# unclearness/vacancy

Measured on AMD Instinct MI355X. Metric: Mvoxel*views/s (Carve), higher is better.
Workload: dtype f32

## Files before the change

vacancy_amd/csrc/carve_fused.h:

```cpp
#pragma once
#include <algorithm>
#include <cstdint>

#include "carve_common.h"
#include "carve_fused_plan.h"

namespace vcy {

constexpr int kMaxFusedViews = 64;
constexpr int kTileRaw = 16;
constexpr int kRawBuffers = 2;
template <int TQ>
constexpr int tile_f4_per_wave() { return TQ == kTileRaw ? kRawBuffers * 64 : TQ; }
constexpr int kTileBig = 512;
constexpr int kBigPixels = 4 * kTileBig;

constexpr int kCoopSdfPitch = 8 * VCY_WG_WAVES + 4;
template <typename CountT>
constexpr int coop_cnt_pitch() { return 8 * VCY_WG_WAVES + 16 / (int)sizeof(CountT); }
template <typename CountT>
constexpr size_t coop_lds_bytes() {
  return 64 * (size_t)kCoopSdfPitch * sizeof(float) + 64 * (size_t)coop_cnt_pitch<CountT>() * sizeof(CountT) +
         2 * VCY_WG_WAVES * sizeof(unsigned long long);
}

template <typename CountT, int NB>
constexpr size_t row_lds_bytes_per_wave() {
  return (size_t)kRawBuffers * 1024 + (size_t)NB * kRowMaxViews * 56  +
         (size_t)NB * 64 * WX * (sizeof(float) + sizeof(CountT)) + (size_t)NB * sizeof(unsigned long long);
}

#ifndef VCY_FAST_GROUP
#define VCY_FAST_GROUP 4
#endif
#ifndef VCY_WAVES
#define VCY_WAVES 7
#endif
#ifndef VCY_WAVES_CHECKED
#define VCY_WAVES_CHECKED 5
#endif
#ifndef VCY_WAVES_WA
#define VCY_WAVES_WA 6
#endif
#ifndef VCY_WAVES_WA_ONE
#define VCY_WAVES_WA_ONE 7
#endif
#ifndef VCY_WAVES_ONE
#define VCY_WAVES_ONE 8
#endif

struct FusedView {
  ViewParams v;
  const float* wmax;
  int wmax_plane;
  int has_lower;
  int wrect[4];
};
constexpr int kC0Stride = 32;

struct TileInfo {
  float lo_x, hi_x, lo_y, hi_y;
  float pitchf;
  int base;
  int tx0, ty0, tw, nq;
  int th;
  float inv_tw;
  float ub;
  int sure;
};
static_assert(sizeof(TileInfo) == 56, "row_lds_bytes_per_wave");

struct FootprintRecord {
  uint32_t w0, w1;
};
static_assert(sizeof(FootprintRecord) == kFootprintRecordBytes, "plan_fused_launch's chunk size");

__device__ __forceinline__ uint32_t pack_footprint_ub(float ub) {
  uint32_t b = __float_as_uint(ub);
  if (!(fabsf(ub) <= 3.402823466e+38f)) b = 0x7f800000u;
  else if (b & 0x80000000u) b &= ~63u;
  else b = (b + 63u) & ~63u;
  return b;
}

__device__ __forceinline__ FootprintRecord pack_footprint(const TileInfo& ti, const ViewParams& v) {
  const uint32_t b = pack_footprint_ub(ti.ub);
  FootprintRecord r;
  const int tx1 = ti.tx0 + ti.tw - 1, ty1 = ti.ty0 + ti.th - 1;
  r.w0 = b | (uint32_t)ti.th | (ti.nq && tx1 == v.roi_max_xi ? 16u : 0u) | (ti.nq && ty1 == v.roi_max_yi ? 32u : 0u);
  r.w1 = ti.nq ? ((uint32_t)ti.tx0 | ((uint32_t)ti.ty0 << 13) | ((uint32_t)ti.tw << 26) | ((uint32_t)ti.sure << 30)) : 0u;
// ... 166 lines not shown
```

vacancy_amd/csrc/carve_fused.hip:

```cpp
#include <algorithm>
#include <cmath>
#include <cstddef>
#include <cstdlib>
#include <cstring>
#include <map>
#include <mutex>
#include <utility>
#include <vector>

#include "carve_fused_device.h"

namespace vcy {
namespace {

constexpr int kWmaxPlanes = 2;


__device__ __forceinline__ void wmax_load8(const float* __restrict__ row, int x0, int w, bool vec, float a[8]) {
#pragma unroll
  for (int j = 0; j < 8; ++j) a[j] = -INFINITY;
  if (row == nullptr) return;
  if (vec) {
    const float4 lo = *(const float4*)(row + x0);
    a[0] = lo.x, a[1] = lo.y, a[2] = lo.z, a[3] = lo.w;
// ... 205 lines not shown
namespace {
__global__ __launch_bounds__(256) void c0_records_kernel(const FusedView* __restrict__ views, const float* __restrict__ px,
                                                         int nx, int nbw, float* __restrict__ c2) {
  const int t = blockIdx.x * 256 + threadIdx.x;
  const int b = t >> 3, k = t & 7;
  if (b >= nbw) return;
  const ViewParams& v = views[blockIdx.y].v;
  const float p = px[min(b * WX + k, nx - 1)];
  float* rec = c2 + ((size_t)blockIdx.y * nbw + b) * kC0Stride;
  rec[2 * k + 0] = v.r[0][0] * p;
  rec[2 * k + 1] = v.r[1][0] * p;
  rec[16 + k] = v.r[2][0] * p;
  rec[24 + k] = 0.0f;
}
}

bool fused_eligible(const vcy_ctx* c, int n_views, const vcy_view* views) {
  const vcy_update_option& u = c->opt.update_option;
  if (count_width_for(c, c->st.views_carved + n_views) > 2) return false;
  if (u.voxel_update == VCY_UPDATE_WEIGHTED_AVERAGE && !sane(u.voxel_update_weight)) return false;
  if (!carve_offsets_fit_32(std::min(n_views, kMaxFusedViews), (c->nx + WX - 1) / WX)) return false;
  for (int i = 0; i < n_views; ++i) {
    const vcy_view& v = views[i];
    if (v.is_ortho != views[0].is_ortho) return false;
    if (!v.is_ortho && (!sane(v.fx) || !sane(v.fy))) return false;
    if (v.width > 8192 || v.height > 8192) return false;
  }
  return true;
}

bool FusedViewCache::matches(const FusedViewKey& k, const void* vp_now, size_t vp_bytes) const {
  return valid && vp.size() == vp_bytes && std::memcmp(vp.data(), vp_now, vp_bytes) == 0 && key == k;
}
void FusedViewCache::remember(const FusedViewKey& k, const void* vp_now, size_t vp_bytes, bool samef_now, int max_quads_now) {
  vp.assign((const char*)vp_now, (const char*)vp_now + vp_bytes);
  key = k, samef = samef_now, max_quads = max_quads_now;
  valid = true;
}

int FusedViewStage::next(size_t bytes, void** out) {
  if (h[1].bytes() < bytes) {
    for (int q = 0; q < 2; ++q) {
      if (ev[q]) (void)hipEventSynchronize(ev[q]);
      (void)h[q].reset();
    }
    const size_t room = bytes + bytes / 2 + 4096;
    for (int q = 0; q < 2; ++q) {
      VCY_HIP_CHECK(ev[q].ensure(hipEventDisableTiming));
      VCY_HIP_CHECK(h[q].alloc(room));
    }
  }
  idx ^= 1;
  VCY_HIP_CHECK(hipEventSynchronize(ev[idx]));
  *out = h[idx];
  return VCY_OK;
}
int FusedViewStage::copied(hipStream_t stream) {
  VCY_HIP_CHECK(hipEventRecord(ev[idx], stream));
  return VCY_OK;
}

struct PreparedViews {
  float* d_c2;
  FusedView* d_views;
  bool samef;
  int max_quads;
};

namespace {

void fill_view_blocks(const vcy_ctx* c, int n_views, const ViewParams* vp, bool ortho, bool need_bound, bool need_lower,
                      int zlo, int zhi, FusedView* fv, bool* samef_out, int* max_quads_out) {
  std::memset((void*)fv, 0, sizeof(FusedView) * (size_t)n_views);
  bool samef = true;
  for (int vi = 0; vi < n_views; ++vi) {
    fv[vi].v = vp[vi];
    samef = samef && (vp[vi].fx == vp[vi].fy);
  }
  int max_quads = 0;
  if (need_bound && c->fused.d_wmax) {
    const int planes = need_lower ? 2 * kWmaxPlanes : kWmaxPlanes;
    const double X[2] = {c->h_px_min, c->h_px_max}, Y[2] = {c->h_py_min, c->h_py_max};
    const double Z[2] = {c->h_pz[zlo], c->h_pz[zhi - 1]};
    size_t off = 0;
    for (int vi = 0; vi < n_views; ++vi) {
      const int npx = vp[vi].width * vp[vi].height;
      fv[vi].wmax = c->fused.d_wmax + off;
      fv[vi].wmax_plane = npx;
      fv[vi].has_lower = need_lower ? 1 : 0;
      off += ((size_t)planes * npx + 3) & ~(size_t)3;
      const ImageRect r = slab_image_rect(vp[vi], ortho, X, Y, Z, vp[vi].width, vp[vi].height);
      for (int i = 0; i < 4; ++i) fv[vi].wrect[i] = r.wrect[i];
      max_quads = std::max(max_quads, r.quads);
    }
  }
  *samef_out = samef, *max_quads_out = max_quads;
}

}

int prepare_views(vcy_ctx* c, int n_views, const ViewParams* vp, bool ortho, bool need_bound, bool need_lower, int zlo,
                  int zhi, PreparedViews* out) {
  FusedState& f = c->fused;
  const int nxp = (c->nx + WX - 1) / WX * WX, nbw = nxp / WX;
  const size_t c2_bytes = (size_t)n_views * nbw * kC0Stride * sizeof(float);
  const size_t fv_bytes = sizeof(FusedView) * (size_t)n_views;
  const size_t vp_bytes = sizeof(ViewParams) * (size_t)n_views;
  if (need_bound) {
    const int planes = need_lower ? 2 * kWmaxPlanes : kWmaxPlanes;
    size_t total = 0;
    for (int vi = 0; vi < n_views; ++vi) total += ((size_t)planes * vp[vi].width * vp[vi].height + 3) & ~(size_t)3;
    if (f.d_wmax.bytes() < total * sizeof(float)) {
      VCY_HIP_CHECK(hipStreamSynchronize(c->stream));
      if (f.d_wmax.alloc(total * sizeof(float)) != hipSuccess) (void)hipGetLastError();
    }
  }
  {
    const size_t had = f.d_scratch.bytes();
    const hipError_t eg = f.d_scratch.grow(c2_bytes + fv_bytes, c->stream);
    if (eg != hipSuccess || f.d_scratch.bytes() != had) f.cache.valid = false;
    VCY_HIP_CHECK(eg);
  }
  float* d_c2 = (float*)f.d_scratch;
  FusedView* d_views = (FusedView*)((char*)f.d_scratch + c2_bytes);
  const FusedViewKey key{f.d_wmax, (void*)d_c2, need_bound, need_lower, ortho, zlo, zhi};
  if (!f.cache.matches(key, vp, vp_bytes)) {
    static_assert(kC0Stride == 32 && WX == 8, "c0_records_kernel's record layout");
    void* stage = nullptr;
    { const int rcs = f.stage.next(fv_bytes, &stage); if (rcs != VCY_OK) return rcs; }
    bool samef = true;
    int max_quads = 0;
    fill_view_blocks(c, n_views, vp, ortho, need_bound, need_lower, zlo, zhi, (FusedView*)stage, &samef, &max_quads);
    VCY_HIP_CHECK(hipMemcpyAsync(d_views, stage, fv_bytes, hipMemcpyHostToDevice, c->stream));
    { const int rcs = f.stage.copied(c->stream); if (rcs != VCY_OK) return rcs; }
    hipLaunchKernelGGL(c0_records_kernel, dim3((unsigned)((nbw * WX + 255) / 256), (unsigned)n_views), dim3(256), 0, c->stream,
                       d_views, c->d_px, c->nx, nbw, d_c2);
    VCY_HIP_CHECK(hipGetLastError());
    f.cache.remember(key, vp, vp_bytes, samef, max_quads);
  }
  out->d_c2 = d_c2;
  out->d_views = d_views;
  out->samef = f.cache.samef;
  out->max_quads = f.cache.max_quads;
  return VCY_OK;
}

void build_window_planes(vcy_ctx* c, const PreparedViews& pv, int n_views, bool need_lower) {
  if (pv.max_quads <= 0) return;
  const dim3 wgrid((unsigned)((pv.max_quads + 255) / 256), (unsigned)n_views);
  hipLaunchKernelGGL(wmax_k4_kernel<false>, wgrid, dim3(256), 0, c->stream, pv.d_views);
  hipLaunchKernelGGL(wmax_k8_kernel<false>, wgrid, dim3(256), 0, c->stream, pv.d_views);
  if (need_lower) {
    hipLaunchKernelGGL(wmax_k4_kernel<true>, wgrid, dim3(256), 0, c->stream, pv.d_views);
    hipLaunchKernelGGL(wmax_k8_kernel<true>, wgrid, dim3(256), 0, c->stream, pv.d_views);
  }
}

namespace {

struct CarveLogScope {
  vcy_ctx* c;
  int n0, last0;
  int stamp = -1;
  bool done = false;
  explicit CarveLogScope(vcy_ctx* ctx) : c(ctx), n0(ctx->carve_log_n), last0(ctx->carve_log_last) {}
  ~CarveLogScope() { if (!done) c->carve_log_n = n0, c->carve_log_last = last0; }
  int open(bool first_chunk) {
    if (!c->time_carve) return VCY_OK;
    stamp = carve_log_open(c, first_chunk);
    return mark(0);
  }
  int mark(int i) {
    if (stamp >= 0) VCY_HIP_CHECK(hipEventRecord(c->carve_log[stamp].ev[i], c->stream));
    return VCY_OK;
  }
};
// ... 168 lines not shown
  { const int rc = log.open(true); if (rc != VCY_OK) return rc; }
  build_window_planes(c, pv, n_views, plan.need_lower);
  if ((int64_t)plan.nbx * plan.nby * plan.nbz > 0x7fffffffLL) {
    set_error("slab too large for one launch");
    return VCY_ERR_TOO_MANY_VOXELS;
  }
  ModeParams m{u.voxel_update, u.sdf_interp, u.update_outside, u.use_truncation ? 1 : 0, ortho ? 1 : 0, 0};
  m.div_level = launch_div_level(c, n_views, vp, ortho);
  c->fused.last_div_level = m.div_level;
  { const int rc = ensure_launch_buffers(c, plan, n_views); if (rc != VCY_OK) return rc; }
  in.have_brick_min = c->d_brick_min != nullptr;
  for (int l0 = 0; l0 < plan.nbz; l0 += plan.chunk_layers) {
    const int layers = std::min(plan.chunk_layers, plan.nbz - l0);
    const ChunkOperands o = chunk_operands(c, g, plan, l0, layers);
    if (l0 > 0) { const int rc = log.open(false); if (rc != VCY_OK) return rc; }
    const FusedChunkPlan chunk = plan_fused_chunk(plan, in, layers, c->fused.h_live_hint, ++c->fused.live_list_age);
    bool reuse = false;
    if (plan.records) {
      const bool have_planes = pv.max_quads > 0;
      const bool cacheable = fused_records_cacheable(plan, in, chunk, have_planes);
      std::vector<char> key;
      if (cacheable) key = record_key(c, plan, pv, n_views, vp, m);
      reuse = fused_reuses_records(plan, in, chunk, have_planes, cacheable && c->fused.rec_cache.matches(key));
      if (reuse) {
        ++c->fused.rec_cache.hits;
      } else {
        const int rc = write_records(c, plan, o, pv, n_views, m, cacheable ? &key : nullptr);
        if (rc != VCY_OK) return rc;
      }
    }
    int live = kLiveNotWaited;
    if (chunk.listed) { const int rc = list_live_workgroups(c, plan, chunk, o, n_views, m.trunc, &live); if (rc != VCY_OK) return rc; }
    FusedChunkLaunch fin = finish_fused_chunk(plan, in, chunk, live);
    if (reuse) fin.state_flags |= kStateStaleBounds;
    { const int rc = launch_chunk(c, plan, chunk, fin, o, pv, n_views, m, &log); if (rc != VCY_OK) return rc; }
  }
  log.done = true;
  c->st.stored();
  c->st.minima_rebuilt(c->d_brick_min != nullptr);
  return VCY_OK;
}

int fused_max_views() { return kMaxFusedViews; }

template <bool SAMEF, bool GEN>
__global__ __launch_bounds__(256) void plan_cost_kernel(GridParams g, const FusedView* __restrict__ views, int nviews,
                                                        int nbw, int nby, int sxn, int syn, int stride, int64_t nsample,
                                                        ModeParams mode, unsigned long long* __restrict__ layer_pairs) {
  const int64_t t = (int64_t)blockIdx.x * 256 + threadIdx.x;
  const bool valid = t < nsample;
  const int64_t tt = valid ? t : nsample - 1;
  const int sx = (int)(tt % sxn);
  const int64_t r = tt / sxn;
  const int sy = (int)(r % syn), bz = (int)(r / syn);
  const int bxw = min(sx * stride + stride / 2, nbw - 1), by = min(sy * stride + stride / 2, nby - 1);
  const int x_lo = min(bxw * WX, g.nx - 1), x_hi = min(bxw * WX + WX - 1, g.nx - 1);
  const int y_hi = min(by * BY + BY - 1, g.ny - 1), z_hi = min(bz * BZ + BZ - 1, g.nz_local - 1);
  const float xl = g.px[x_lo], xh = g.px[x_hi], yl = g.py[by * BY], yh = g.py[y_hi];
  const float zl = g.pz[g.z0 + bz * BZ], zh = g.pz[g.z0 + z_hi];
  const bool update_max = mode.update == VCY_UPDATE_MAX;
  float smin = -INFINITY;
  bool touched = false;
  int count = 0;
  for (int vi = 0; vi < nviews; ++vi) {
    float lb = -INFINITY;
    const TileInfo ti = footprint_of<SAMEF, kTileRaw, GEN>(views[vi], xl, xh, yl, yh, zl, zh, mode.ortho != 0,
                                                            mode.outside == VCY_OUTSIDE_MAX, true, true, &lb);
// ... 99 lines not shown
```

vacancy_amd/csrc/carve_fused_device.h:

```cpp
#pragma once
#include "carve_fused.h"

namespace vcy {
namespace {

#define VCY_SETPRIO(n) __builtin_amdgcn_s_setprio(n)

#ifdef VCY_PHASE_TIMING
__device__ unsigned long long g_phase_ticks[256][16];
#define VCY_PT_DECL unsigned long long pt_last = __builtin_amdgcn_s_memtime(), pt_acc[16] = {0, 0, 0, 0, 0, 0, 0, 0, 0, 0, 0, 0, 0, 0, 0, 0}
#define VCY_PT(slot)                                                  \
  do {                                                                \
    const unsigned long long t_ = __builtin_amdgcn_s_memtime();       \
    pt_acc[slot] += t_ - pt_last;                                     \
    pt_last = t_;                                                     \
  } while (0)
#define VCY_PT_COUNT(slot) pt_acc[slot] += 1
#define VCY_PT_FLUSH(lane_)                                                                         \
  do {                                                                                              \
    if ((lane_) == 0)                                                                               \
      for (int q_ = 0; q_ < 16; ++q_) atomicAdd(&g_phase_ticks[blockIdx.x & 255][q_], pt_acc[q_]);  \
  } while (0)
#else
#define VCY_PT_DECL
// ... 278 lines not shown
  const int tx0 = __builtin_amdgcn_readfirstlane(ti.tx0);
  const int ty0 = __builtin_amdgcn_readfirstlane(ti.ty0);
  const float inv_pitch = __uint_as_float(__builtin_amdgcn_readfirstlane(__float_as_uint(ti.inv_tw)));
  const int pitch = tw + 1, npx = pitch * (th + 1);
  gfloat_ptr img = (gfloat_ptr)v.sdf;
  const unsigned width = (unsigned)v.width;
  lds_float* dst = (lds_float*)tile;
  for (int q0 = 0; q0 < npx; q0 += 64) {
    const int q = q0 + lane;
    if (q < npx) {
      const int j = div_small(q, inv_pitch), i = q - j * pitch;
      const unsigned xx = (unsigned)min(tx0 + i, v.roi_max_xi), yy = (unsigned)min(ty0 + j, v.roi_max_yi);
      __builtin_amdgcn_global_load_lds(img + (__umul24(width, yy) + xx), dst + q0, 4, 0, 0);
    }
  }
  raw_tile_wait();
}

struct FootprintWindows {
  int pw, ph;
  int L;
  int nxw, nyw;
};
__device__ __forceinline__ FootprintWindows footprint_windows(int tx0, int ty0, int tx1, int ty1, int roi_max_xi,
                                                              int roi_max_yi) {
  FootprintWindows fw;
  fw.pw = min(tx1 + 1, roi_max_xi) - tx0 + 1;
  fw.ph = min(ty1 + 1, roi_max_yi) - ty0 + 1;
  fw.L = min(fw.pw, fw.ph) >= 8 ? 3 : 2;
  const int k = 1 << fw.L;
  fw.nxw = (fw.pw + k - 1) >> fw.L, fw.nyw = (fw.ph + k - 1) >> fw.L;
  return fw;
}
template <bool EXACT_COUNTS = true>
__device__ __forceinline__ void footprint_window_requests(gfloat_ptr wm, unsigned width, unsigned plane_off, int tx0, int ty0,
                                                          const FootprintWindows& fw, float t[9]) {
  const int L = fw.L, k = 1 << L, pw = fw.pw, ph = fw.ph;
  const unsigned origin = __umul24(width, (unsigned)ty0) + (unsigned)tx0 + plane_off;
#pragma unroll
  for (int q = 0; q < 9; ++q) t[q] = -INFINITY;
  const bool small = fw.nxw <= 3 && fw.nyw <= 3;
  int ux, uy;
  if (EXACT_COUNTS) {
    ux = __any(small && fw.nxw >= 3) ? 3 : (__any(small && fw.nxw >= 2) ? 2 : 1);
    uy = __any(small && fw.nyw >= 3) ? 3 : (__any(small && fw.nyw >= 2) ? 2 : 1);
  } else {
    ux = uy = __any(small && (fw.nxw >= 3 || fw.nyw >= 3)) ? 3 : 2;
  }
  if (small) {
    auto look = [&](int aq, int bq) {
      const unsigned ro = origin + __umul24(width, (unsigned)min(bq << L, max(ph - k, 0)));
      t[3 * bq + aq] = load_u32_index(wm, ro + (unsigned)min(aq << L, max(pw - k, 0)));
    };
    if (EXACT_COUNTS) {
#pragma unroll
      for (int bq = 0; bq < 3; ++bq) {
#pragma unroll
        for (int aq = 0; aq < 3; ++aq)
          if (aq < ux && bq < uy) look(aq, bq);
      }
    } else {
      look(0, 0), look(1, 0), look(0, 1), look(1, 1);
      if (ux == 3) look(2, 0), look(2, 1), look(0, 2), look(1, 2), look(2, 2);
    }
  } else {
    float m = -INFINITY;
    for (int bq = 0; bq < fw.nyw; ++bq) {
      const unsigned ro = origin + __umul24(width, (unsigned)min(bq << L, max(ph - k, 0)));
      for (int aq = 0; aq < fw.nxw; ++aq) m = fmaxf(m, load_u32_index(wm, ro + (unsigned)min(aq << L, max(pw - k, 0))));
    }
    t[0] = m;
  }
}
__device__ __forceinline__ float footprint_window_max(const float t[9]) {
  float m = -INFINITY;
#pragma unroll
  for (int q = 0; q < 9; ++q) m = fmaxf(m, t[q]);
  return m;
}
__device__ __forceinline__ float footprint_upper_bound(float m, int has_nan, bool outside_max, bool sure, float max_sdf) {
  if (outside_max && !sure) {
    has_nan |= !(fabsf(max_sdf) <= 3.402823466e+38f);
    m = fmaxf(m, max_sdf);
  }
  return has_nan ? INFINITY : (__builtin_fmaf(fabsf(m), 0x1p-20f, m) + 1.0e-30f);
}

template <bool SAMEF, int TQ, bool GEN>
__device__ __forceinline__ TileInfo footprint_of(const FusedView& fv, float xl, float xh, float yl, float yh, float zl_,
                                                 float zh, bool is_ortho, bool outside_max, bool want_bound,
                                                 bool want_lower, float* lower_out = nullptr) {
  const ViewParams& v = fv.v;
  const float xa = fmaxf(fabsf(xl), fabsf(xh)), ya = fmaxf(fabsf(yl), fabsf(yh)), za = fmaxf(fabsf(zl_), fabsf(zh));
  const bool ortho = GEN && is_ortho;
  float p0[3], ax[3], ay[3], az[3], mag[3];
#pragma unroll
  for (int i = 0; i < 3; ++i) {
    p0[i] = v.t[i] + (v.r[i][0] * xl + (v.r[i][1] * yl + v.r[i][2] * zl_));
// ... 108 lines not shown
        }
        ti.ub = footprint_upper_bound(m, has_nan, outside_max, ti.sure != 0, v.max_sdf);
        if (want_lower && ti.sure && !(ti.ub < -1.0f) && wm != nullptr && fv.has_lower && fw.nxw <= 3 && fw.nyw <= 3) {
          float t[9];
          footprint_window_requests(wm, (unsigned)v.width, (L == 3 ? 3u : 2u) * (unsigned)fv.wmax_plane, tx0, ty0, fw, t);
          const float mneg = footprint_window_max(t);
          const float neg_lb = __builtin_fmaf(fabsf(mneg), 0x1p-20f, mneg);
          if (neg_lb <= 1.0f) ti.sure |= 2;
          if (lower_out) *lower_out = -neg_lb;
        }
      }
    }
  }
  return ti;
}

__device__ __forceinline__ FusedView load_fused_view(const FusedView* __restrict__ views, int vi) {
  static_assert(sizeof(FusedView) % 4 == 0, "FusedView is fetched dword by dword");
  constexpr int kViewDwords = (int)(sizeof(FusedView) / 4);
  typedef const uint32_t __attribute__((address_space(1))) * gu32_ptr;
  gu32_ptr src = (gu32_ptr)views + (size_t)vi * kViewDwords;
  uint32_t raw[kViewDwords];
#pragma unroll
  for (int q = 0; q < kViewDwords; ++q) raw[q] = src[q];
#pragma unroll
  for (int q = 0; q < kViewDwords; ++q) asm volatile("" : "+v"(raw[q]));
  FusedView fv;
  __builtin_memcpy(&fv, raw, sizeof(FusedView));
  return fv;
}

struct BoundView {
  gfloat_ptr wmax;
  unsigned wmax_plane, width;
  int roi_max_xi, roi_max_yi;
  float max_sdf;
};
__device__ __forceinline__ BoundView load_bound_view(const FusedView* __restrict__ views, int vi) {
  typedef const char __attribute__((address_space(1))) * gchar_ptr;
  typedef const FusedView __attribute__((address_space(1))) * gview_ptr;
  const FusedView __attribute__((address_space(1)))& fv = *(gview_ptr)((gchar_ptr)views + view_byte_offset(vi));
  BoundView b;
  b.wmax = (gfloat_ptr)fv.wmax;
  b.wmax_plane = (unsigned)fv.wmax_plane, b.width = (unsigned)fv.v.width;
  b.roi_max_xi = fv.v.roi_max_xi, b.roi_max_yi = fv.v.roi_max_yi;
  b.max_sdf = fv.v.max_sdf;
  return b;
}

__device__ __forceinline__ void store_tile_info(lds_u32* tinfo_lds, int vi, const TileInfo& ti) {
  static_assert(sizeof(TileInfo) % 4 == 0, "TileInfo is stored dword by dword");
  uint32_t w32[sizeof(TileInfo) / 4];
  __builtin_memcpy(w32, &ti, sizeof(TileInfo));
  lds_u32* dst = tinfo_lds + vi * (int)(sizeof(TileInfo) / 4);
#pragma unroll
  for (int q = 0; q < (int)(sizeof(TileInfo) / 4); ++q) dst[q] = w32[q];
}

template <bool SAMEF, int TQ, bool GEN>
__device__ __attribute__((noinline)) float brick_footprints(const FusedView* __restrict__ views, int nviews, int lane,
                                                            float xl, float xh, float yl, float yh, float zl_, float zh,
                                                            bool is_ortho, bool outside_max, bool want_bound,
                                                            bool want_lower, lds_u32* tinfo_lds) {
  float ub_lane = INFINITY;
  if (lane < nviews) {
    const FusedView fv = load_fused_view(views, lane);
    const TileInfo ti = footprint_of<SAMEF, TQ, GEN>(fv, xl, xh, yl, yh, zl_, zh, is_ortho, outside_max, want_bound,
                                                     want_lower);
    store_tile_info(tinfo_lds, lane, ti);
    ub_lane = ti.ub;
  }
  return ub_lane;
}

template <bool SAMEF, bool GEN>
__device__ __attribute__((noinline)) FootprintRecord brick_footprint_records(const FusedView* __restrict__ views, int nviews,
                                                                             int lane, float xl, float xh, float yl, float yh,
                                                                             float zl_, float zh, bool is_ortho,
                                                                             bool outside_max, bool want_bound,
// ... 15 lines not shown
```

vacancy_amd/csrc/carve_fused_kernel.h:

```cpp
#pragma once
#include <cstddef>
#include <cstdio>
#include <cstdlib>
#include <type_traits>

#include "carve_fused_device.h"

namespace vcy {
namespace {

template <int UPDATE, bool CHECKMAX, int TQ, bool GEN, int NB>
constexpr int carve_waves_per_simd() {
  if (NB > 1) return NB > 2 ? 4 : 5;
  if (GEN || CHECKMAX || TQ != kTileRaw || UPDATE == VCY_UPDATE_WEIGHTED_AVERAGE) return VCY_WAVES_CHECKED;
  if (UPDATE == kUpdateWaUnitWeight) return NB == 0 ? VCY_WAVES_WA_ONE : VCY_WAVES_WA;
  return NB == 0 ? VCY_WAVES_ONE : VCY_WAVES;
}
template <int UPDATE, int TQ, int NB>
constexpr bool carve_keeps_records() {
  return UPDATE == VCY_UPDATE_MAX && TQ == kTileRaw && NB == 1;
}
template <typename CountT, int UPDATE, bool TRUNC, bool SAMEF, bool CHECKMAX, int TQ, bool GEN, int DIV, int NB = 1>
__global__ __launch_bounds__(64 * (NB > 1 ? kRowWaves : kWgWaves))
__attribute__((amdgpu_waves_per_eu(NB > 1 ? 1 : carve_waves_per_simd<UPDATE, CHECKMAX, TQ, GEN, NB>(),
// ... 158 lines not shown
    asm volatile("" ::"v"(py), "v"(pz));
    const unsigned long long t_ = __builtin_amdgcn_s_memtime();
    pt_acc[12] += t_ - pt_last;
  }
#endif
  const int pair_j = lane >> 3, pair_v = lane & 7;
  const bool pair_valid = kRows && pair_j < NB && pair_v < nviews && x_seg + pair_j * WX < g.nx;
  if constexpr (kRows) {
    ub_lane = INFINITY;
    if (pair_valid) {
      typedef uint32_t u32x2 __attribute__((ext_vector_type(2)));
      typedef const u32x2 __attribute__((address_space(1))) * grec_ptr;
      const u32x2 raw = ((grec_ptr)records)[(int64_t)pair_v * nbricks + (brick_seg + pair_j)];
      FootprintRecord rec;
      rec.w0 = raw.x, rec.w1 = raw.y;
      const TileInfo ti = unpack_footprint(rec);
      store_tile_info((lds_u32*)tinfo, lane, ti);
      ub_lane = ti.ub;
    }
  } else if constexpr (kOneRegs) {
    typedef uint32_t u32x2 __attribute__((ext_vector_type(2)));
    typedef const u32x2 __attribute__((address_space(1))) * grec_ptr;
    FootprintRecord rec;
    if (list_entry != nullptr) {
      rec = list_rec;
    } else {
      const u32x2 raw = ((grec_ptr)records)[brick_lin];
      rec.w0 = (uint32_t)__builtin_amdgcn_readfirstlane((int)raw.x), rec.w1 = (uint32_t)__builtin_amdgcn_readfirstlane((int)raw.y);
    }
    ti_one = unpack_footprint(rec);
    ub_lane = ti_one.ub;
  } else if (kRecRegs && stale_bounds) {
    if constexpr (kRecRegs) {
      typedef uint32_t u32x2 __attribute__((ext_vector_type(2)));
      typedef const u32x2 __attribute__((address_space(1))) * grec_ptr;
      ub_lane = INFINITY;
      const bool has_view = lane < nviews;
      const int lv = has_view ? lane : 0;
      typedef const char __attribute__((address_space(1))) * gchar_ptr;
      static_assert(kRecordBytesMax <= ((int64_t)1 << 31), "the records' byte offset is formed in 32 bits");
      u32x2 raw = *(grec_ptr)((gchar_ptr)records + (((uint32_t)lv * (uint32_t)nbricks + (uint32_t)brick_lin) << 3));
      BoundView bv = load_bound_view(views, lv);
      asm volatile("" : "+v"(raw.x), "+v"(raw.y), "+v"(bv.wmax), "+v"(bv.wmax_plane), "+v"(bv.width), "+v"(bv.roi_max_xi),
                   "+v"(bv.roi_max_yi), "+v"(bv.max_sdf));
      if (has_view) rec_w0 = footprint_ub_word(raw.x, raw.y), rec_w1 = footprint_tile_word(raw.x, raw.y);
      if (fresh && !TRUNC) {
        vi_stale = 0;
        prefetch_tile(0, raw_buf(0));
      }
      const int tw = (int)((raw.y >> 26) & 15u), th = (int)(raw.x & 15u);
      if (has_view && tw != 0) {
        const int tx0 = (int)(raw.y & 8191u), ty0 = (int)((raw.y >> 13) & 8191u);
        const FootprintWindows fw = footprint_windows(tx0, ty0, tx0 + tw - 1, ty0 + th - 1, bv.roi_max_xi, bv.roi_max_yi);
        float t[9];
        footprint_window_requests<false>(bv.wmax, bv.width, fw.L == 3 ? bv.wmax_plane : 0u, tx0, ty0, fw, t);
        const float ub = footprint_upper_bound(footprint_window_max(t), 0, mode.outside == VCY_OUTSIDE_MAX,
                                               ((raw.y >> 30) & 1u) != 0u, bv.max_sdf);
        rec_w0 = pack_footprint_ub(ub) | (raw.x & 63u);
      }
    }
  } else if (kRaw && records != nullptr) {
    ub_lane = INFINITY;
    if (lane < nviews) {
      typedef uint32_t u32x2 __attribute__((ext_vector_type(2)));
      typedef const u32x2 __attribute__((address_space(1))) * grec_ptr;
      const u32x2 raw = ((grec_ptr)records)[(int64_t)lane * nbricks + brick_lin];
      if constexpr (kRecRegs) {
        rec_w0 = footprint_ub_word(raw.x, raw.y), rec_w1 = footprint_tile_word(raw.x, raw.y);
      } else {
        FootprintRecord rec;
        rec.w0 = raw.x, rec.w1 = raw.y;
        const TileInfo ti = unpack_footprint(rec);
        store_tile_info((lds_u32*)tinfo, lane, ti);
        ub_lane = ti.ub;
      }
    }
  } else if constexpr (kRecRegs) {
    const int x_lo = min(x_first, g.nx - 1), x_hi = min(x_first + WX - 1, g.nx - 1);
    const int y_hi = min(by * BY + BY - 1, g.ny - 1);
    const int z_hi = min(zl0 + BZ - 1, g.nz_local - 1);
    const FootprintRecord rec = brick_footprint_records<SAMEF, GEN>(
        views, nviews, lane, g.px[x_lo], g.px[x_hi], g.py[by * BY], g.py[y_hi], g.pz[g.z0 + zl0], g.pz[g.z0 + z_hi],
        mode.ortho != 0, mode.outside == VCY_OUTSIDE_MAX, want_bound, want_bound && TRUNC && UPDATE != VCY_UPDATE_MAX);
    rec_w0 = footprint_ub_word(rec.w0, rec.w1), rec_w1 = footprint_tile_word(rec.w0, rec.w1);
    ub_lane = INFINITY;
  } else {
    const int x_lo = min(x_first, g.nx - 1), x_hi = min(x_first + WX - 1, g.nx - 1);
    const int y_hi = min(by * BY + BY - 1, g.ny - 1);
    const int z_hi = min(zl0 + BZ - 1, g.nz_local - 1);
    ub_lane = brick_footprints<SAMEF, TQ, GEN>(views, nviews, lane, g.px[x_lo], g.px[x_hi], g.py[by * BY], g.py[y_hi],
                                               g.pz[g.z0 + zl0], g.pz[g.z0 + z_hi], mode.ortho != 0,
// ... 867 lines not shown
```

vacancy_amd/csrc/carve_fused_plan.h:

```cpp
#pragma once

#include <algorithm>
#include <cmath>
#include <cstddef>
#include <cstdint>

#include "vacancy_hip.h"

namespace vcy {

#ifndef VCY_WG_WAVES
#define VCY_WG_WAVES 4
#endif
constexpr int kWgWaves = VCY_WG_WAVES;
constexpr int BX = 8 * kWgWaves, BY = 8, BZ = 8;
constexpr int WX = 8;
constexpr int kRowMaxViews = 8;
#ifndef VCY_ROW_BRICKS
#define VCY_ROW_BRICKS 4
#endif
#ifndef VCY_ROW_WAVES
#define VCY_ROW_WAVES 2
#endif
constexpr int kRowBricks = VCY_ROW_BRICKS;
constexpr int kRowWaves = VCY_ROW_WAVES;
constexpr int kLiveListMaxViews = 8;
constexpr int kLiveEntryWords = 2 + 2 * kWgWaves;
constexpr int64_t kRecordBytesMax = (int64_t)2 << 30;
constexpr int kFootprintRecordBytes = 8;

constexpr int kUpdateWaUnitWeight = 2;

constexpr int kStateFresh = 1;
constexpr int kStateCountImplied = 2;
constexpr int kStateBrickMinValid = 4;
constexpr int kStateCoopStore = 8;
constexpr int kStateStreamStore = 16;
constexpr int kStateEager = 32;
constexpr int kStateListRecords = 64;
constexpr int kStateStaleBounds = 128;

enum class CarveFlavour {
  kGeneral,
  kOneView,
  kRows,
};

struct FusedKnobs {
  int tile_mode = 0;
  int row_kernel = 0;
  int one_view = 1;
  int coop_store = -1;
  int nt_store = -1;
  int prologue_mode = 0;
  int64_t record_bytes_max = 0;
  bool use_live_list = true;
  int list_records = 1;
  int eager_state = -1;
  bool live_sync = true;
  bool use_cull = true;
  bool count_pairs = false;
  bool use_short_div = true;
  bool record_cache = true;
};

struct FusedPlanInput {
  int update = VCY_UPDATE_MAX;
  bool trunc = false;
  int interp = VCY_INTERP_BILINEAR;
  int64_t max_update_num = 255;
  float weight = 1.0f;
  int nx = 0, ny = 0, nz_local = 0;
  bool fresh = false, cnt_implied = true, brick_min_valid = false;
// ... 125 lines not shown
}

struct FusedChunkLaunch {
  unsigned grid_x;
  bool eager_state;
  int state_flags;
};
constexpr int kLiveNotWaited = -1;

inline FusedChunkLaunch finish_fused_chunk(const FusedLaunchPlan& p, const FusedPlanInput& in, const FusedChunkPlan& c,
                                           int live) {
  FusedChunkLaunch f;
  f.grid_x = c.listed ? c.listed_grid : c.full_grid;
  if (c.listed && live >= 0 && live <= c.units) f.grid_x = fused_groups_of(p, (unsigned)live);
  const bool nearly_all_live = c.listed ? f.grid_x < (unsigned)c.units || !c.list_pays : !c.list_pays;
  f.eager_state = !in.fresh && p.one_view && (in.knobs.eager_state > 0 || (in.knobs.eager_state < 0 && nearly_all_live));
  f.state_flags = p.state_flags_base | (f.eager_state ? kStateEager : 0) |
                  (c.listed && c.list_entry_words ? kStateListRecords : 0);
  return f;
}

inline bool fused_records_cacheable(const FusedLaunchPlan& p, const FusedPlanInput& in, const FusedChunkPlan& c,
                                    bool have_planes) {
  const bool keeps_records = p.update == VCY_UPDATE_MAX && !p.big && p.flavour == CarveFlavour::kGeneral;
  return in.knobs.record_cache && keeps_records && p.need_bound && !p.want_lower &&
         p.records  && p.chunk_layers >= p.nbz && have_planes &&
         !c.listed ;
}
inline bool fused_reuses_records(const FusedLaunchPlan& p, const FusedPlanInput& in, const FusedChunkPlan& c,
                                 bool have_planes, bool key_matches) {
  return fused_records_cacheable(p, in, c, have_planes) && key_matches;
}

struct ImageRect {
  int wrect[4];
  int quads;
};
template <class View>
inline ImageRect slab_image_rect(const View& v, bool ortho, const double X[2], const double Y[2], const double Z[2], int w,
                                 int h) {
  int rx0 = 0, ry0 = 0, rx1 = w, ry1 = h;
  double umin = 1e300, umax = -1e300, wmin = 1e300, wmax = -1e300;
  bool whole = false;
  for (int cr = 0; cr < 8; ++cr) {
    const double x = X[cr & 1], y = Y[(cr >> 1) & 1], z = Z[cr >> 2];
    double pc[3];
    for (int i = 0; i < 3; ++i)
      pc[i] = (double)v.t[i] + ((double)v.r[i][0] * x + (double)v.r[i][1] * y + (double)v.r[i][2] * z);
    double uu = pc[0], ww = pc[1];
    if (!ortho) {
      if (!(pc[2] > 1e-30)) { whole = true; break; }
      uu = (double)v.fx / pc[2] * pc[0] + v.cx;
      ww = (double)v.fy / pc[2] * pc[1] + v.cy;
    }
    if (!(std::fabs(uu) < 1e9) || !(std::fabs(ww) < 1e9)) { whole = true; break; }
    umin = std::min(umin, uu), umax = std::max(umax, uu);
    wmin = std::min(wmin, ww), wmax = std::max(wmax, ww);
  }
  if (!whole) {
    rx0 = std::max(0, (int)std::floor(umin) - 16) & ~3;
    ry0 = std::max(0, (int)std::floor(wmin) - 16);
    rx1 = std::min((w + 3) & ~3, ((int)std::floor(umax) + 16 + 4) & ~3);
    ry1 = std::min(h, (int)std::floor(wmax) + 16 + 1);
    if (rx1 < rx0) rx1 = rx0;
    if (ry1 < ry0) ry1 = ry0;
  } else {
// ... 7 lines not shown
```

vacancy_amd/csrc/carve_fused_state.h:

```cpp
#pragma once

#include <cstddef>
#include <cstdint>
#include <utility>
#include <vector>

#include "carve_fused_plan.h"
#include "vcy_resources.h"

namespace vcy {

struct FusedViewKey {
  const float* wmax;
  const void* at;
  bool bound, lower, ortho;
  int zlo, zhi;
  bool operator==(const FusedViewKey& o) const {
    return wmax == o.wmax && at == o.at && bound == o.bound && lower == o.lower && ortho == o.ortho && zlo == o.zlo &&
           zhi == o.zhi;
  }
};
struct FusedViewCache {
  bool valid = false;
  std::vector<char> vp;
  FusedViewKey key{};
  bool samef = true;
  int max_quads = 0;
  bool matches(const FusedViewKey& k, const void* vp_now, size_t vp_bytes) const;
  void remember(const FusedViewKey& k, const void* vp_now, size_t vp_bytes, bool samef_now, int max_quads_now);
};

struct FusedRecordCache {
  bool valid = false;
  std::vector<char> key;
  int hits = 0;
  bool matches(const std::vector<char>& k) const { return valid && key == k; }
  void remember(std::vector<char>&& k) { key = std::move(k), valid = true; }
  void forget() { valid = false; }
};

struct FusedViewStage {
  PinnedBuf<> h[2];
  Event ev[2];
  int idx = 0;
  int next(size_t bytes, void** out);
  int copied(hipStream_t stream);
};

struct FusedState {
  FusedKnobs knobs;
  FusedViewCache cache;
  FusedViewStage stage;
  DeviceBuf<> d_scratch;
  DeviceBuf<float> d_wmax;
  DeviceBuf<> d_records;
  FusedRecordCache rec_cache;
  DeviceBuf<int> d_wg_list;
  PinnedBuf<int> h_live_hint;
  int64_t live_list_age = 0;
  DeviceBuf<unsigned long long> d_pair_count;
  int pair_count_views = 0;
  int last_div_level = 0;
// ... 8 lines not shown
```

Measured before the change: 4.854 million.

## Add SoA bound table and split stale-bound refresh across two half-waves

Adds a structure-of-arrays table of per-view bound fields (plane offset, plane size, width, ROI limits, max SDF) behind the view blocks. When records are reused with stale bounds, lanes read it with coalesced dword loads, and the wmax base pointer comes from a single scalar load. When there are at most 32 views, each view's footprint window lookups are split across two lanes (lane and lane+32), and the partial maxima are combined with a permlane32 swap. This targets the latency of the strided AoS gathers and of the serial window loads in the bound-refresh prologue, at the cost of extra host table filling, a larger upload and more code paths.

```diff
diff --git a/vacancy_amd/csrc/carve_fused.h b/vacancy_amd/csrc/carve_fused.h
--- a/vacancy_amd/csrc/carve_fused.h
+++ b/vacancy_amd/csrc/carve_fused.h
@@ -56,6 +56,16 @@
   int has_lower;
   int wrect[4];
 };
+#ifndef VCY_DEV_BOUND_TABLE
+#define VCY_DEV_BOUND_TABLE 1
+#endif
+#ifndef VCY_DEV_BOUND_TWO_LANES
+#define VCY_DEV_BOUND_TWO_LANES 1
+#endif
+static_assert(kBoundTableViews == kMaxFusedViews, "a slot per view of the largest launch, a lane per slot");
+static_assert(sizeof(FusedView) % 4 == 0, "the table behind the view blocks is dword aligned");
+__host__ __device__ __forceinline__ uint32_t bound_table_byte_offset(int n_views) { return (uint32_t)n_views * (uint32_t)sizeof(FusedView); }
+
 constexpr int kC0Stride = 32;
 
 struct TileInfo {
diff --git a/vacancy_amd/csrc/carve_fused.hip b/vacancy_amd/csrc/carve_fused.hip
--- a/vacancy_amd/csrc/carve_fused.hip
+++ b/vacancy_amd/csrc/carve_fused.hip
@@ -261,9 +261,10 @@
 bool FusedViewCache::matches(const FusedViewKey& k, const void* vp_now, size_t vp_bytes) const {
   return valid && vp.size() == vp_bytes && std::memcmp(vp.data(), vp_now, vp_bytes) == 0 && key == k;
 }
-void FusedViewCache::remember(const FusedViewKey& k, const void* vp_now, size_t vp_bytes, bool samef_now, int max_quads_now) {
+void FusedViewCache::remember(const FusedViewKey& k, const void* vp_now, size_t vp_bytes, bool samef_now, int max_quads_now,
+                              int64_t plane_span_now) {
   vp.assign((const char*)vp_now, (const char*)vp_now + vp_bytes);
-  key = k, samef = samef_now, max_quads = max_quads_now;
+  key = k, samef = samef_now, max_quads = max_quads_now, plane_span = plane_span_now;
   valid = true;
 }
 
@@ -292,6 +293,7 @@
 struct PreparedViews {
   float* d_c2;
   FusedView* d_views;
+  int64_t plane_span;
   bool samef;
   int max_quads;
 };
@@ -299,7 +301,7 @@
 namespace {
 
 void fill_view_blocks(const vcy_ctx* c, int n_views, const ViewParams* vp, bool ortho, bool need_bound, bool need_lower,
-                      int zlo, int zhi, FusedView* fv, bool* samef_out, int* max_quads_out) {
+                      int zlo, int zhi, FusedView* fv, bool* samef_out, int* max_quads_out, int64_t* plane_span_out) {
   std::memset((void*)fv, 0, sizeof(FusedView) * (size_t)n_views);
   bool samef = true;
   for (int vi = 0; vi < n_views; ++vi) {
@@ -324,6 +326,8 @@
     }
   }
   *samef_out = samef, *max_quads_out = max_quads;
+  *plane_span_out = fill_bound_table(fv, n_views, need_lower ? 2 * kWmaxPlanes : kWmaxPlanes,
+                                     (uint32_t*)((char*)fv + bound_table_byte_offset(n_views)));
 }
 
 }
@@ -333,7 +337,7 @@
   FusedState& f = c->fused;
   const int nxp = (c->nx + WX - 1) / WX * WX, nbw = nxp / WX;
   const size_t c2_bytes = (size_t)n_views * nbw * kC0Stride * sizeof(float);
-  const size_t fv_bytes = sizeof(FusedView) * (size_t)n_views;
+  const size_t fv_bytes = sizeof(FusedView) * (size_t)n_views + sizeof(uint32_t) * kBoundTableWords;
   const size_t vp_bytes = sizeof(ViewParams) * (size_t)n_views;
   if (need_bound) {
     const int planes = need_lower ? 2 * kWmaxPlanes : kWmaxPlanes;
@@ -359,18 +363,20 @@
     { const int rcs = f.stage.next(fv_bytes, &stage); if (rcs != VCY_OK) return rcs; }
     bool samef = true;
     int max_quads = 0;
-    fill_view_blocks(c, n_views, vp, ortho, need_bound, need_lower, zlo, zhi, (FusedView*)stage, &samef, &max_quads);
+    int64_t plane_span = 0;
+    fill_view_blocks(c, n_views, vp, ortho, need_bound, need_lower, zlo, zhi, (FusedView*)stage, &samef, &max_quads, &plane_span);
     VCY_HIP_CHECK(hipMemcpyAsync(d_views, stage, fv_bytes, hipMemcpyHostToDevice, c->stream));
     { const int rcs = f.stage.copied(c->stream); if (rcs != VCY_OK) return rcs; }
     hipLaunchKernelGGL(c0_records_kernel, dim3((unsigned)((nbw * WX + 255) / 256), (unsigned)n_views), dim3(256), 0, c->stream,
                        d_views, c->d_px, c->nx, nbw, d_c2);
     VCY_HIP_CHECK(hipGetLastError());
-    f.cache.remember(key, vp, vp_bytes, samef, max_quads);
+    f.cache.remember(key, vp, vp_bytes, samef, max_quads, plane_span);
   }
   out->d_c2 = d_c2;
   out->d_views = d_views;
   out->samef = f.cache.samef;
   out->max_quads = f.cache.max_quads;
+  out->plane_span = f.cache.plane_span;
   return VCY_OK;
 }
 
@@ -605,7 +611,7 @@
     int live = kLiveNotWaited;
     if (chunk.listed) { const int rc = list_live_workgroups(c, plan, chunk, o, n_views, m.trunc, &live); if (rc != VCY_OK) return rc; }
     FusedChunkLaunch fin = finish_fused_chunk(plan, in, chunk, live);
-    if (reuse) fin.state_flags |= kStateStaleBounds;
+    if (reuse) fin.state_flags |= fused_stale_bound_flags(pv.plane_span);
     { const int rc = launch_chunk(c, plan, chunk, fin, o, pv, n_views, m, &log); if (rc != VCY_OK) return rc; }
   }
   log.done = true;
diff --git a/vacancy_amd/csrc/carve_fused_device.h b/vacancy_amd/csrc/carve_fused_device.h
--- a/vacancy_amd/csrc/carve_fused_device.h
+++ b/vacancy_amd/csrc/carve_fused_device.h
@@ -334,9 +334,10 @@
   fw.nxw = (fw.pw + k - 1) >> fw.L, fw.nyw = (fw.ph + k - 1) >> fw.L;
   return fw;
 }
+constexpr int kAllRows = -1;
 template <bool EXACT_COUNTS = true>
 __device__ __forceinline__ void footprint_window_requests(gfloat_ptr wm, unsigned width, unsigned plane_off, int tx0, int ty0,
-                                                          const FootprintWindows& fw, float t[9]) {
+                                                          const FootprintWindows& fw, float t[9], int half = kAllRows) {
   const int L = fw.L, k = 1 << L, pw = fw.pw, ph = fw.ph;
   const unsigned origin = __umul24(width, (unsigned)ty0) + (unsigned)tx0 + plane_off;
 #pragma unroll
@@ -350,10 +351,11 @@
     ux = uy = __any(small && (fw.nxw >= 3 || fw.nyw >= 3)) ? 3 : 2;
   }
   if (small) {
-    auto look = [&](int aq, int bq) {
+    auto window = [&](int aq, int bq) -> float {
       const unsigned ro = origin + __umul24(width, (unsigned)min(bq << L, max(ph - k, 0)));
-      t[3 * bq + aq] = load_u32_index(wm, ro + (unsigned)min(aq << L, max(pw - k, 0)));
+      return load_u32_index(wm, ro + (unsigned)min(aq << L, max(pw - k, 0)));
     };
+    auto look = [&](int aq, int bq) { t[3 * bq + aq] = window(aq, bq); };
     if (EXACT_COUNTS) {
 #pragma unroll
       for (int bq = 0; bq < 3; ++bq) {
@@ -361,11 +363,14 @@
         for (int aq = 0; aq < 3; ++aq)
           if (aq < ux && bq < uy) look(aq, bq);
       }
+    } else if (half != kAllRows) {
+      t[0] = window(0, half), t[1] = window(1, half);
+      if (ux == 3) t[2] = window(2, half), t[3] = window(2 * half, 2), t[4] = window(1 + half, 2);
     } else {
       look(0, 0), look(1, 0), look(0, 1), look(1, 1);
       if (ux == 3) look(2, 0), look(2, 1), look(0, 2), look(1, 2), look(2, 2);
     }
-  } else {
+  } else if (half <= 0) {
     float m = -INFINITY;
     for (int bq = 0; bq < fw.nyw; ++bq) {
       const unsigned ro = origin + __umul24(width, (unsigned)min(bq << L, max(ph - k, 0)));
@@ -540,19 +545,34 @@
 
 struct BoundView {
   gfloat_ptr wmax;
-  unsigned wmax_plane, width;
+  unsigned plane, wmax_plane, width;
   int roi_max_xi, roi_max_yi;
   float max_sdf;
 };
-__device__ __forceinline__ BoundView load_bound_view(const FusedView* __restrict__ views, int vi) {
+template <bool TABLE>
+__device__ __forceinline__ BoundView load_bound_view(const FusedView* __restrict__ views, int n_views, int slot) {
   typedef const char __attribute__((address_space(1))) * gchar_ptr;
-  typedef const FusedView __attribute__((address_space(1))) * gview_ptr;
-  const FusedView __attribute__((address_space(1)))& fv = *(gview_ptr)((gchar_ptr)views + view_byte_offset(vi));
   BoundView b;
-  b.wmax = (gfloat_ptr)fv.wmax;
-  b.wmax_plane = (unsigned)fv.wmax_plane, b.width = (unsigned)fv.v.width;
-  b.roi_max_xi = fv.v.roi_max_xi, b.roi_max_yi = fv.v.roi_max_yi;
-  b.max_sdf = fv.v.max_sdf;
+  if constexpr (TABLE) {
+    typedef const uint32_t __attribute__((address_space(1))) * gu32_ptr;
+    typedef const FusedView __attribute__((address_space(4))) * cview_ptr;
+    gu32_ptr tab = (gu32_ptr)((gchar_ptr)views + bound_table_byte_offset(n_views));
+    auto word = [&](int field) -> uint32_t {
+      return *(gu32_ptr)((gchar_ptr)tab + (((uint32_t)slot << 2) + (uint32_t)(field * kBoundTableViews * 4)));
+    };
+    b.wmax = (gfloat_ptr)((cview_ptr)views)->wmax;
+    b.plane = word(kBoundPlane), b.wmax_plane = word(kBoundPlaneSize), b.width = word(kBoundWidth);
+    b.roi_max_xi = (int)word(kBoundRoiMaxX), b.roi_max_yi = (int)word(kBoundRoiMaxY);
+    b.max_sdf = __uint_as_float(word(kBoundMaxSdf));
+  } else {
+    typedef const FusedView __attribute__((address_space(1))) * gview_ptr;
+    const FusedView __attribute__((address_space(1)))& fv = *(gview_ptr)((gchar_ptr)views + view_byte_offset(slot));
+    b.wmax = (gfloat_ptr)fv.wmax;
+    b.plane = 0u;
+    b.wmax_plane = (unsigned)fv.wmax_plane, b.width = (unsigned)fv.v.width;
+    b.roi_max_xi = fv.v.roi_max_xi, b.roi_max_yi = fv.v.roi_max_yi;
+    b.max_sdf = fv.v.max_sdf;
+  }
   return b;
 }
 
diff --git a/vacancy_amd/csrc/carve_fused_kernel.h b/vacancy_amd/csrc/carve_fused_kernel.h
--- a/vacancy_amd/csrc/carve_fused_kernel.h
+++ b/vacancy_amd/csrc/carve_fused_kernel.h
@@ -214,31 +214,62 @@
     ub_lane = ti_one.ub;
   } else if (kRecRegs && stale_bounds) {
     if constexpr (kRecRegs) {
-      typedef uint32_t u32x2 __attribute__((ext_vector_type(2)));
-      typedef const u32x2 __attribute__((address_space(1))) * grec_ptr;
       ub_lane = INFINITY;
-      const bool has_view = lane < nviews;
-      const int lv = has_view ? lane : 0;
-      typedef const char __attribute__((address_space(1))) * gchar_ptr;
-      static_assert(kRecordBytesMax <= ((int64_t)1 << 31), "the records' byte offset is formed in 32 bits");
-      u32x2 raw = *(grec_ptr)((gchar_ptr)records + (((uint32_t)lv * (uint32_t)nbricks + (uint32_t)brick_lin) << 3));
-      BoundView bv = load_bound_view(views, lv);
-      asm volatile("" : "+v"(raw.x), "+v"(raw.y), "+v"(bv.wmax), "+v"(bv.wmax_plane), "+v"(bv.width), "+v"(bv.roi_max_xi),
-                   "+v"(bv.roi_max_yi), "+v"(bv.max_sdf));
-      if (has_view) rec_w0 = footprint_ub_word(raw.x, raw.y), rec_w1 = footprint_tile_word(raw.x, raw.y);
-      if (fresh && !TRUNC) {
-        vi_stale = 0;
-        prefetch_tile(0, raw_buf(0));
-      }
-      const int tw = (int)((raw.y >> 26) & 15u), th = (int)(raw.x & 15u);
-      if (has_view && tw != 0) {
-        const int tx0 = (int)(raw.y & 8191u), ty0 = (int)((raw.y >> 13) & 8191u);
-        const FootprintWindows fw = footprint_windows(tx0, ty0, tx0 + tw - 1, ty0 + th - 1, bv.roi_max_xi, bv.roi_max_yi);
-        float t[9];
-        footprint_window_requests<false>(bv.wmax, bv.width, fw.L == 3 ? bv.wmax_plane : 0u, tx0, ty0, fw, t);
-        const float ub = footprint_upper_bound(footprint_window_max(t), 0, mode.outside == VCY_OUTSIDE_MAX,
-                                               ((raw.y >> 30) & 1u) != 0u, bv.max_sdf);
-        rec_w0 = pack_footprint_ub(ub) | (raw.x & 63u);
+      auto refresh_bounds = [&](auto table_c, auto two_c) {
+        constexpr bool kTable = decltype(table_c)::value, kTwo = decltype(two_c)::value;
+        typedef uint32_t u32x2 __attribute__((ext_vector_type(2)));
+        typedef const u32x2 __attribute__((address_space(1))) * grec_ptr;
+        const int slot = kTwo ? (lane & 31) : lane, half = kTwo ? (lane >> 5) : kAllRows;
+        const bool has_view = slot < nviews;
+        const bool packs = lane < nviews;
+        const int lv = has_view ? slot : 0;
+        typedef const char __attribute__((address_space(1))) * gchar_ptr;
+        static_assert(kRecordBytesMax <= ((int64_t)1 << 31), "the records' byte offset is formed in 32 bits");
+        u32x2 raw = *(grec_ptr)((gchar_ptr)records + (((uint32_t)lv * (uint32_t)nbricks + (uint32_t)brick_lin) << 3));
+        BoundView bv = load_bound_view<kTable>(views, nviews, kTable ? slot : lv);
+        if constexpr (kTable)
+          asm volatile("" : "+v"(raw.x), "+v"(raw.y), "+v"(bv.plane), "+v"(bv.wmax_plane), "+v"(bv.width), "+v"(bv.roi_max_xi),
+                       "+v"(bv.roi_max_yi), "+v"(bv.max_sdf));
+        else
+          asm volatile("" : "+v"(raw.x), "+v"(raw.y), "+v"(bv.wmax), "+v"(bv.wmax_plane), "+v"(bv.width), "+v"(bv.roi_max_xi),
+                       "+v"(bv.roi_max_yi), "+v"(bv.max_sdf));
+        if (packs) rec_w0 = footprint_ub_word(raw.x, raw.y), rec_w1 = footprint_tile_word(raw.x, raw.y);
+        if (fresh && !TRUNC) {
+          vi_stale = 0;
+          prefetch_tile(0, raw_buf(0));
+        }
+        const int tw = (int)((raw.y >> 26) & 15u), th = (int)(raw.x & 15u);
+        const bool bounds = has_view && tw != 0;
+        float m = -INFINITY;
+        if (bounds) {
+          const int tx0 = (int)(raw.y & 8191u), ty0 = (int)((raw.y >> 13) & 8191u);
+          const FootprintWindows fw = footprint_windows(tx0, ty0, tx0 + tw - 1, ty0 + th - 1, bv.roi_max_xi, bv.roi_max_yi);
+          float t[9];
+          footprint_window_requests<false>(bv.wmax, bv.width, bv.plane + (fw.L == 3 ? bv.wmax_plane : 0u), tx0, ty0, fw, t, half);
+          m = footprint_window_max(t);
+        }
+        if constexpr (kTwo) {
+          const auto sw = __builtin_amdgcn_permlane32_swap(__float_as_uint(m), __float_as_uint(m), false, false);
+          m = fmaxf(__uint_as_float(sw[0]), __uint_as_float(sw[1]));
+        }
+        if (bounds && packs) {
+          const float ub = footprint_upper_bound(m, 0, mode.outside == VCY_OUTSIDE_MAX, ((raw.y >> 30) & 1u) != 0u, bv.max_sdf);
+          rec_w0 = pack_footprint_ub(ub) | (raw.x & 63u);
+        }
+      };
+      constexpr bool kDevTable = VCY_DEV_BOUND_TABLE != 0, kDevTwo = VCY_DEV_BOUND_TWO_LANES != 0;
+      const bool table = kDevTable && (state_flags & kStateBoundTable) != 0;
+      const bool two = kDevTwo && nviews <= 32;
+      if (table) {
+        if (two) refresh_bounds(std::true_type{}, std::true_type{});
+        else refresh_bounds(std::true_type{}, std::false_type{});
+      } else {
+        if constexpr (!kDevTable) {
+          if (two) refresh_bounds(std::false_type{}, std::true_type{});
+          else refresh_bounds(std::false_type{}, std::false_type{});
+        } else {
+          refresh_bounds(std::false_type{}, std::false_type{});
+        }
       }
     }
   } else if (kRaw && records != nullptr) {
diff --git a/vacancy_amd/csrc/carve_fused_plan.h b/vacancy_amd/csrc/carve_fused_plan.h
--- a/vacancy_amd/csrc/carve_fused_plan.h
+++ b/vacancy_amd/csrc/carve_fused_plan.h
@@ -4,6 +4,7 @@
 #include <cmath>
 #include <cstddef>
 #include <cstdint>
+#include <cstring>
 
 #include "vacancy_hip.h"
 
@@ -39,6 +40,7 @@
 constexpr int kStateEager = 32;
 constexpr int kStateListRecords = 64;
 constexpr int kStateStaleBounds = 128;
+constexpr int kStateBoundTable = 256;
 
 enum class CarveFlavour {
   kGeneral,
@@ -230,6 +232,40 @@
   return fused_records_cacheable(p, in, c, have_planes) && key_matches;
 }
 
+enum BoundField { kBoundPlane = 0, kBoundPlaneSize, kBoundWidth, kBoundRoiMaxX, kBoundRoiMaxY, kBoundMaxSdf, kBoundFields };
+constexpr int kBoundTableViews = 64;
+constexpr int kBoundTableWords = kBoundFields * kBoundTableViews;
+constexpr int64_t kBoundPlaneSpanMax = (int64_t)1 << 32;
+
+template <class FV>
+inline int64_t fill_bound_table(const FV* fv, int n_views, int planes, uint32_t* table) {
+  std::memset(table, 0, sizeof(uint32_t) * kBoundTableWords);
+  int64_t span = 0;
+  for (int vi = 0; vi < n_views && vi < kBoundTableViews; ++vi) {
+    uint32_t* slot = table + vi;
+    int64_t first = 0;
+    if (fv[vi].wmax != nullptr && fv[0].wmax != nullptr) {
+      first = ((int64_t)(uintptr_t)fv[vi].wmax - (int64_t)(uintptr_t)fv[0].wmax) / (int64_t)sizeof(float);
+      span = std::max(span, (first + (int64_t)planes * fv[vi].wmax_plane) * (int64_t)sizeof(float));
+      if (first < 0) span = kBoundPlaneSpanMax + 1;
+    }
+    slot[kBoundPlane * kBoundTableViews] = (uint32_t)(uint64_t)first;
+    slot[kBoundPlaneSize * kBoundTableViews] = (uint32_t)fv[vi].wmax_plane;
+    slot[kBoundWidth * kBoundTableViews] = (uint32_t)fv[vi].v.width;
+    slot[kBoundRoiMaxX * kBoundTableViews] = (uint32_t)fv[vi].v.roi_max_xi;
+    slot[kBoundRoiMaxY * kBoundTableViews] = (uint32_t)fv[vi].v.roi_max_yi;
+    const float ms = fv[vi].v.max_sdf;
+    std::memcpy(&slot[kBoundMaxSdf * kBoundTableViews], &ms, sizeof(uint32_t));
+  }
+  return span;
+}
+inline bool bound_planes_fit_32(int64_t plane_span_bytes) {
+  return plane_span_bytes > 0 && plane_span_bytes <= kBoundPlaneSpanMax;
+}
+inline int fused_stale_bound_flags(int64_t plane_span_bytes) {
+  return kStateStaleBounds | (bound_planes_fit_32(plane_span_bytes) ? kStateBoundTable : 0);
+}
+
 struct ImageRect {
   int wrect[4];
   int quads;
diff --git a/vacancy_amd/csrc/carve_fused_state.h b/vacancy_amd/csrc/carve_fused_state.h
--- a/vacancy_amd/csrc/carve_fused_state.h
+++ b/vacancy_amd/csrc/carve_fused_state.h
@@ -26,8 +26,10 @@
   FusedViewKey key{};
   bool samef = true;
   int max_quads = 0;
+  int64_t plane_span = 0;
   bool matches(const FusedViewKey& k, const void* vp_now, size_t vp_bytes) const;
-  void remember(const FusedViewKey& k, const void* vp_now, size_t vp_bytes, bool samef_now, int max_quads_now);
+  void remember(const FusedViewKey& k, const void* vp_now, size_t vp_bytes, bool samef_now, int max_quads_now,
+                int64_t plane_span_now);
 };
 
 struct FusedRecordCache {
```

After: 4.849 million (median of 3 runs). Within noise of the previous version (-0.1%).
